# Lymphatus/caesium-clt

Measured on NVIDIA H100. Metric: megapixels/sec JPEG q=80 4K re-encode, higher is better.
Workload: dtype i32

## Files before the change

### caesium-clt_b200/csrc/jpeg_gpuenc.cu

```cuda
#include <cuda_runtime.h>
#include <cub/device/device_scan.cuh>
#include <cuda_pipeline.h>
#include <algorithm>
#include <chrono>
#include <cstring>
#include "jpeg_gpuenc.h"
#include "stream_wait.h"
#include "launch_timer.h"

namespace b200 {

using namespace ge;

__global__ void k_ge_groups(const Scan *__restrict__ scans, const uint32_t *__restrict__ meta, const int *__restrict__ evkey,
                            const int *__restrict__ prev, const uint32_t *__restrict__ tsum, uint32_t *__restrict__ gcount, uint32_t *__restrict__ hist)
{
    __shared__ uint32_t eob[16];
    const Scan s = scans[blockIdx.y];
    if (s.mode != MODE_AC_FIRST && s.mode != MODE_AC_REFINE) return;
    if ((int)(blockIdx.x * blockDim.x) > s.nblocks) return;
    if (threadIdx.x < 16) eob[threadIdx.x] = 0;
    __syncthreads();
    const int b = blockIdx.x * blockDim.x + threadIdx.x;
    if (b <= s.nblocks && (b == s.nblocks || meta_event(meta[s.unit_base + b]))) {
        int pg;
        if (b < s.nblocks) pg = prev[s.unit_base + b];
        else { const long long last = s.unit_base + s.nblocks - 1; pg = max(prev[last], evkey[last]); }
        const int pl = pg >= s.unit_base ? (int)(pg - s.unit_base) : -1;
        assign_groups(meta + s.unit_base, tsum + s.unit_base, s.nblocks, pl, b, gcount + s.unit_base,
                      [&](uint32_t c) { atomicAdd(&eob[eob_symbol(c) >> 4], 1u); });
    }
    __syncthreads();
    if (threadIdx.x < 16 && eob[threadIdx.x]) atomicAdd(&hist[((size_t)s.tab_base + 2 + s.tbl[0]) * 256 + (threadIdx.x << 4)], eob[threadIdx.x]);
}

__global__ void k_ge_tables(const uint32_t *__restrict__ hist, Table *__restrict__ tabs, DhtOut *__restrict__ dht, unsigned long long *__restrict__ tbits)
{
    __shared__ long long freq[257];
    __shared__ int codesize[257], others[257];
    __shared__ uint8_t bits[33];
    const int t = blockIdx.x, lane = threadIdx.x;
    const uint32_t *f = hist + (size_t)t * 256;
    for (int i = lane; i < 257; i += 32) { freq[i] = i < 256 ? (long long)f[i] : 1; codesize[i] = 0; others[i] = -1; }
    if (lane == 0) for (int i = 0; i < 33; i++) bits[i] = 0;
    __syncwarp();
    auto warp_argmin = [&](int exclude) {
        unsigned long long v = 1000000000ULL; int c = -1;
        for (int i = lane; i < 257; i += 32) { const unsigned long long fi = (unsigned long long)freq[i]; if (fi && fi <= v && i != exclude) { v = fi; c = i; } }
        const unsigned hi = (unsigned)(v >> 32), lo = (unsigned)v;
        const unsigned mhi = __reduce_min_sync(0xFFFFFFFFu, hi);
        const unsigned mlo = __reduce_min_sync(0xFFFFFFFFu, hi == mhi ? lo : 0xFFFFFFFFu);
        return __reduce_max_sync(0xFFFFFFFFu, (hi == mhi && lo == mlo) ? c : -1);
    };
    for (;;) {
        const int c1 = warp_argmin(-1);
        const int c2 = c1 < 0 ? -1 : warp_argmin(c1);
        if (c2 < 0) break;
        if (lane == 0) {
            int a = c1, b = c2;
            freq[a] += freq[b]; freq[b] = 0;
            codesize[a]++; while (others[a] >= 0) { a = others[a]; codesize[a]++; }
            others[a] = b;
            codesize[b]++; while (others[b] >= 0) { b = others[b]; codesize[b]++; }
        }
        __syncwarp();
    }
    if (lane == 0) {
        Table &T = tabs[t];
        for (int i = 0; i <= 256; i++) if (codesize[i]) bits[codesize[i] > 32 ? 32 : codesize[i]]++;
        for (int i = 32; i > 16; i--) while (bits[i] > 0) {
            int j = i - 2; while (bits[j] == 0) j--;
            bits[i] -= 2; bits[i - 1]++; bits[j + 1] += 2; bits[j]--;
        }
        int i = 16; while (i > 0 && bits[i] == 0) i--;
        if (i > 0) bits[i]--;
        int start[34];
        for (int l = 0; l < 34; l++) start[l] = 0;
        for (int s = 0; s <= 255; s++) if (codesize[s]) start[min(codesize[s], 32) + 1]++;
        for (int l = 1; l < 34; l++) start[l] += start[l - 1];
        const int p = start[33];
        for (int s = 0; s <= 255; s++) if (codesize[s]) T.vals[start[min(codesize[s], 32)]++] = (uint8_t)s;
        T.nvals = p;
        for (int k = 0; k < 17; k++) T.bits[k] = bits[k];
        for (int s = 0; s < 256; s++) T.code_len[s] = 0;
        uint32_t code = 0; int k = 0;
        for (int l = 1; l <= 16; l++) { for (int n = 0; n < bits[l]; n++, k++) T.code_len[T.vals[k]] = (code++ << 8) | (uint32_t)l; code <<= 1; }
        DhtOut &D = dht[t];
        D.nvals = p;
        for (int k2 = 0; k2 < 17; k2++) D.bits[k2] = bits[k2];
        for (int k2 = 0; k2 < p; k2++) D.vals[k2] = T.vals[k2];
    }
    __syncwarp();
    const int kind = (t & 3) >> 1;
    unsigned long long nb = 0;
    for (int i = lane; i < 256; i += 32) if (f[i]) nb += (unsigned long long)f[i] * ((tabs[t].code_len[i] & 0xFFu) + (unsigned)sym_extra_bits(kind, i));
    for (int d = 16; d; d >>= 1) nb += __shfl_xor_sync(0xFFFFFFFFu, nb, d);
    if (lane == 0) tbits[t] = nb;
}

__global__ void k_ge_scanout(const Scan *__restrict__ scans, int nscans, const unsigned long long *__restrict__ tbits, const uint32_t *__restrict__ corr,
                             uint32_t *__restrict__ total, ScanOut *__restrict__ so, uint32_t words_cap, uint32_t groups_cap, uint32_t *__restrict__ flags)
{
    const int lane = threadIdx.x;
    uint32_t wbase = 0, gbase = 0, abase = 0;
    for (int c0 = 0; c0 < nscans; c0 += 32) {
        const int i = c0 + lane;
        uint32_t tb = 0, na = 0;
        if (i < nscans) {
            tb = (uint32_t)(tbits[4 * i] + tbits[4 * i + 1] + tbits[4 * i + 2] + tbits[4 * i + 3] + corr[i]);
            na = scans[i].nruns ? (tb + 31) / 32 + scans[i].nruns : 0;
        }
        const uint32_t nbytes = (tb + 7) / 8, ng = (nbytes + 15) / 16, nw = i < nscans ? (tb + 31) / 32 + 1 : 0;
        uint32_t wi = nw, gi = i < nscans ? ng : 0, ai = na;
        for (int d = 1; d < 32; d <<= 1) {
            const uint32_t a = __shfl_up_sync(0xFFFFFFFFu, wi, d), b = __shfl_up_sync(0xFFFFFFFFu, gi, d), c = __shfl_up_sync(0xFFFFFFFFu, ai, d);
            if (lane >= d) { wi += a; gi += b; ai += c; }
        }
        if (i < nscans) {
            total[i] = tb;
            ScanOut o; o.total_bits = tb; o.nbytes = nbytes; o.ngroups = ng; o.group_base = gbase + gi - ng; o.word_base = wbase + wi - nw; o.arena_base = abase + ai - na;
            so[i] = o;
        }
        wbase += __shfl_sync(0xFFFFFFFFu, wi, 31); gbase += __shfl_sync(0xFFFFFFFFu, gi, 31); abase += __shfl_sync(0xFFFFFFFFu, ai, 31);
    }
    __syncwarp();
    const bool ovf = wbase > words_cap || gbase > groups_cap;
    if (lane == 0) { flags[0] = ovf ? 1u : 0u; flags[1] = wbase; flags[2] = gbase; flags[3] = 0; flags[4] = 0; }
    if (ovf) for (int i = lane; i < nscans; i += 32) { so[i].total_bits = 0; so[i].nbytes = 0; so[i].ngroups = 0; so[i].group_base = 0; so[i].word_base = 0; so[i].arena_base = 0; }
}

__global__ void k_ge_zero(const Scan *__restrict__ scans, const ScanOut *__restrict__ so, uint32_t *__restrict__ words, uint32_t *__restrict__ arena)
{
    const ScanOut o = so[blockIdx.y];
    if (!o.total_bits) return;
    const uint32_t n = (o.total_bits + 31) / 32 + 1, nruns = (uint32_t)scans[blockIdx.y].nruns, na = nruns ? n - 1 + nruns : 0;
    uint32_t *w = words + o.word_base, *a = arena + o.arena_base;
    for (uint32_t i = blockIdx.x * blockDim.x + threadIdx.x; i < max(n, na); i += gridDim.x * blockDim.x) {
        if (i < n) w[i] = 0;
        if (i < na) a[i] = 0;
    }
}

constexpr int TILE_PITCH = 72;
typedef int16_t Tile[ENC_THREADS][TILE_PITCH];

__device__ __forceinline__ void stage_tile(Tile &tile, const BlockComp &bc, int i0, int nblk)
{
    const uint4 *src = reinterpret_cast<const uint4 *>(bc.coef + bc.comp_off + (long long)i0 * 64);
    const int n = min(ENC_THREADS, nblk - i0) * 8;
#pragma unroll
    for (int k = 0; k < 8; k++) { const int q = threadIdx.x + k * ENC_THREADS; if (q < n) __pipeline_memcpy_async(&tile[q >> 3][(q & 7) * 8], src + q, 16); }
    __pipeline_commit();
}
__device__ __forceinline__ void wait_tile()
{
    __pipeline_wait_prior(0);
    __syncthreads();
}

__device__ __forceinline__ void stage_visits(EncVisit *vis, const BlockComp &bc)
{
    if ((int)threadIdx.x < bc.nscan) vis[threadIdx.x] = bc.visit[threadIdx.x];
}
__device__ __forceinline__ BlockRef ref_of(const EncVisit &v, const BlockComp &bc, const Tile &tile, int i0, int row, int col)
{
    BlockRef r;
    r.blk = tile[threadIdx.x]; r.prev = nullptr; r.slot = 0;
    if (v.mode == MODE_SEQ || v.mode == MODE_DC_FIRST) {
        const int p = enc_dc_prev(bc, v.ns, row, col);
        if (p >= i0 && p < i0 + ENC_THREADS) r.prev = tile[p - i0];
        else if (p >= 0) r.prev = bc.coef + bc.comp_off + (long long)p * 64;
    }
    return r;
}

template <class T>
__device__ __forceinline__ KindTabs<T> kind_tabs(T *tab, const EncVisit &v) { return KindTabs<T>{tab + ENC_DC_ENTRY, tab + v.ac_entry}; }

__device__ __forceinline__ Masks3 load_masks(const Masks3 *__restrict__ masks, const BlockComp &bc, int i)
{
    const unsigned long long *q = reinterpret_cast<const unsigned long long *>(masks + bc.mask_base + i);
    Masks3 M;
    M.m[0] = __ldg(q); M.m[1] = __ldg(q + 1); M.m[2] = __ldg(q + 2);
    return M;
}

struct SmemHist {
    KindTabs<uint32_t> h;
    __device__ void sym(int kind, int, int symbol, int, unsigned) { atomicAdd((kind ? h.ac : h.dc) + symbol, 1u); }
    __device__ void raw64(int, unsigned long long) {}
};
__global__ void __launch_bounds__(ENC_THREADS) k_geb_classify(const BlockComp *__restrict__ comps, uint32_t *__restrict__ meta, int *__restrict__ evkey,
                                                              uint32_t *__restrict__ tail, Masks3 *__restrict__ masks, uint32_t *__restrict__ hist, uint32_t *__restrict__ corr)
{
    __shared__ __align__(16) Tile tile;
    __shared__ uint32_t h[ENC_TAB_ENTRIES];
    __shared__ EncVisit vis[ENC_MAX_VISITS];
    __shared__ uint32_t vcorr[ENC_MAX_VISITS];
    const BlockComp &bc = comps[blockIdx.y];
    const int nblk = bc.bw * bc.bh, i0 = blockIdx.x * ENC_THREADS, i = i0 + threadIdx.x;
    if (i0 >= nblk) return;
    stage_tile(tile, bc, i0, nblk);
    for (int k = threadIdx.x; k < ENC_TAB_ENTRIES; k += ENC_THREADS) h[k] = 0;
    if (threadIdx.x < ENC_MAX_VISITS) vcorr[threadIdx.x] = 0;
    stage_visits(vis, bc);
    wait_tile();
    if (i < nblk) {
        const int row = i / bc.bw, col = i - row * bc.bw;
        const Masks3 M = make_masks3(tile[threadIdx.x]);
        masks[bc.mask_base + i] = M;
        for (int j = 0; j < bc.nscan; j++) {
// ... 86 lines not shown
                                                          const uint32_t *__restrict__ flags, uint32_t *__restrict__ arena, uint32_t *__restrict__ cursor,
                                                          uint32_t *__restrict__ runlen, uint32_t *__restrict__ runpos)
{
    __shared__ __align__(16) Tile tile;
    __shared__ uint32_t tc[ENC_TAB_ENTRIES];
    __shared__ EncVisit vis[ENC_MAX_VISITS];
    __shared__ uint32_t vword[ENC_MAX_VISITS], vbit0[ENC_MAX_VISITS];
    __shared__ uint32_t slot[ENC_SLOT_WORDS][ENC_THREADS];
    __shared__ uint32_t wsum[ENC_THREADS / 32], run_word;
    if (flags[0]) return;
    const BlockComp &bc = comps[blockIdx.y];
    const int nblk = bc.bw * bc.bh, i0 = blockIdx.x * ENC_THREADS, i = i0 + threadIdx.x;
    if (i0 >= nblk) return;
    const bool live = i < nblk;
    stage_tile(tile, bc, i0, nblk);
    const Masks3 M = load_masks(masks, bc, min(i, nblk - 1));
    stage_visits(vis, bc);
    if ((int)threadIdx.x < bc.nscan) {
        const EncVisit &v = bc.visit[threadIdx.x];
        const ScanOut &o = so[v.scan];
        vword[threadIdx.x] = v.ns > 1 ? o.word_base : o.arena_base; vbit0[threadIdx.x] = v.ns > 1 ? bitoff[v.lu_base] : 0;
    }
    for (int k = threadIdx.x; k < ENC_TAB_ENTRIES; k += ENC_THREADS) {
        int symbol; const int t = enc_entry_table(bc, k, symbol);
        if (t >= 0) tc[k] = tabs[t].code_len[symbol];
    }
    wait_tile();
    const int row = i / bc.bw, col = i - row * bc.bw;
    auto orw = [&](long long w, uint32_t v) { if (v) atomicOr(&words[w], v); };
    auto stw = [&](long long w, uint32_t v) { words[w] = v; };
    auto ora = [&](long long w, uint32_t v) { if (v) atomicOr(&arena[w], v); };
    auto sta = [&](long long w, uint32_t v) { arena[w] = v; };
    auto sls = [&](long long w, uint32_t v) { if (w < ENC_SLOT_WORDS) slot[w][threadIdx.x] = v; };
    typedef KindTabs<const uint32_t> KT;
    for (int j = 0; j < bc.nscan; j++) {
        const EncVisit &v = vis[j];
        const int u = live ? enc_unit_of(bc, v.ns, row, col) : -1;
        if (v.ns > 1) {
            if (u < 0) continue;
            EmitSink<decltype(orw), decltype(stw), KT> sk(kind_tabs<const uint32_t>(tc, v), orw, stw, (long long)vword[j], (unsigned long long)(bitoff[v.lu_base + u] - vbit0[j]));
            gen_block_m(v, v.tbl, ref_of(v, bc, tile, i0, row, col), M, gcount[v.unit_base + u], sk);
            sk.finish();
            continue;
        }
        uint32_t nb = 0;
        if (u >= 0) {
            EmitSink<decltype(sls), decltype(sls), KT> sk(kind_tabs<const uint32_t>(tc, v), sls, sls, 0, 0);
            gen_block_m(v, v.tbl, ref_of(v, bc, tile, i0, row, col), M, gcount[v.unit_base + u], sk);
            sk.finish();
            nb = (uint32_t)sk.bits_written(0);
        }
        uint32_t L;
        const uint32_t off = cta_exclusive_sum(nb, wsum, L);
        if (threadIdx.x == 0) {
            const uint32_t a = vword[j] + atomicAdd(&cursor[v.scan], (L + 31) / 32);
            run_word = a; runlen[v.run_base + blockIdx.x] = L; runpos[v.run_base + blockIdx.x] = a;
        }
        __syncthreads();
        const unsigned long long at = (unsigned long long)run_word * 32 + off;
        if (nb <= ENC_SLOT_WORDS * 32) place_bits([&](long long k) { return slot[k][threadIdx.x]; }, nb, at, ora, sta);
        else {
            EmitSink<decltype(ora), decltype(sta), KT> sk(kind_tabs<const uint32_t>(tc, v), ora, sta, 0, at);
            gen_block_m(v, v.tbl, ref_of(v, bc, tile, i0, row, col), M, gcount[v.unit_base + u], sk);
            sk.finish();
        }
    }
}

constexpr int PLACE_THREADS = 128;
__global__ void __launch_bounds__(PLACE_THREADS) k_ge_place(const Scan *__restrict__ scans, const ScanOut *__restrict__ so, const uint32_t *__restrict__ runlen,
                                                            const uint32_t *__restrict__ runoff, const uint32_t *__restrict__ runpos, const uint32_t *__restrict__ arena,
                                                            uint32_t *__restrict__ words, const uint32_t *__restrict__ flags)
{
    if (flags[0]) return;
    const int nruns = scans[blockIdx.y].nruns, x = blockIdx.x * (PLACE_THREADS / 32) + (threadIdx.x >> 5);
    if (x >= nruns) return;
    const int r0 = scans[blockIdx.y].run_base, r = r0 + x;
    const uint32_t *src = arena + runpos[r];
    uint32_t *dst = words + so[blockIdx.y].word_base;
    place_bits([&](long long k) { return src[k]; }, runlen[r], runoff[r] - runoff[r0],
               [&](long long w, uint32_t v) { atomicOr(&dst[w], v); }, [&](long long w, uint32_t v) { dst[w] = v; }, threadIdx.x & 31, 32);
}

__device__ __forceinline__ uint32_t scan_byte(const uint32_t *__restrict__ w, uint32_t i, uint32_t nbytes, uint32_t total_bits)
{
    uint32_t b = (w[i >> 2] >> (24 - 8 * (i & 3))) & 0xFF;
    if (i == nbytes - 1 && (total_bits & 7)) b |= (1u << (8 - (total_bits & 7))) - 1u;
    return b;
}

__global__ void k_ge_ffcount(const ScanOut *__restrict__ so, int nscans, const uint32_t *__restrict__ words, uint32_t *__restrict__ ffcount, uint32_t groups_cap,
                             const uint32_t *__restrict__ flags)
{
    if ((int)blockIdx.y == nscans) {
        const uint32_t used = flags[0] ? 0u : flags[2];
        for (uint32_t g = used + blockIdx.x * blockDim.x + threadIdx.x; g < groups_cap; g += gridDim.x * blockDim.x) ffcount[g] = 0;
        return;
    }
    const ScanOut o = so[blockIdx.y];
    const uint32_t *w = words + o.word_base;
    for (uint32_t g = blockIdx.x * blockDim.x + threadIdx.x; g < o.ngroups; g += gridDim.x * blockDim.x) {
        uint32_t n = 0;
        for (uint32_t i = g * 16; i < g * 16 + 16 && i < o.nbytes; i++) n += scan_byte(w, i, o.nbytes, o.total_bits) == 0xFF;
        ffcount[o.group_base + g] = n;
    }
}

__global__ void k_ge_layout(const ScanOut *__restrict__ so, int scans_per_image, int nimages, const uint32_t *__restrict__ ffcount, const uint32_t *__restrict__ ffoff,
                            uint32_t *__restrict__ out_off, uint32_t *__restrict__ out_len, uint32_t out_image_stride, uint32_t *__restrict__ flags)
{
    const int im = blockIdx.x * blockDim.x + threadIdx.x;
    if (im >= nimages) return;
    uint32_t off = 0;
    for (int k = 0; k < scans_per_image; k++) {
        const int si = im * scans_per_image + k;
        const ScanOut o = so[si];
        uint32_t ff = 0;
        if (o.ngroups) { const uint32_t lastg = o.group_base + o.ngroups - 1; ff = ffoff[lastg] + ffcount[lastg] - ffoff[o.group_base]; }
        out_off[si] = off; out_len[si] = o.nbytes + ff;
        off += o.nbytes + ff;
    }
    atomicMax(&flags[3], off);
    if (off > out_image_stride) atomicOr(&flags[4], 1u);
}

__global__ void k_ge_scatter(const ScanOut *__restrict__ so, const uint32_t *__restrict__ words, const uint32_t *__restrict__ ffoff,
                             const uint32_t *__restrict__ out_off, uint8_t *__restrict__ out, int scans_per_image, size_t out_image_stride, const uint32_t *__restrict__ flags)
{
    if (flags[4]) return;
    const ScanOut o = so[blockIdx.y];
    const uint32_t *w = words + o.word_base;
    uint8_t *base = out + (size_t)(blockIdx.y / scans_per_image) * out_image_stride + out_off[blockIdx.y];
    for (uint32_t g = blockIdx.x * blockDim.x + threadIdx.x; g < o.ngroups; g += gridDim.x * blockDim.x) {
        uint8_t *dst = base + (size_t)g * 16 + (ffoff[o.group_base + g] - ffoff[o.group_base]);
        for (uint32_t i = g * 16; i < g * 16 + 16 && i < o.nbytes; i++) {
            const uint32_t b = scan_byte(w, i, o.nbytes, o.total_bits);
            *dst++ = (uint8_t)b;
            if (b == 0xFF) *dst++ = 0;
        }
    }
}

__global__ void k_ge_fill_dummy(int16_t *__restrict__ coef, long long comp_off, int bw, int bh, int rbw, int rbh, int hs)
{
    const int i = blockIdx.x * blockDim.x + threadIdx.x;
    if (i >= bw * bh) return;
    const int row = i / bw, col = i - row * bw;
    if (row < rbh && col < rbw) return;
    int r = row, c = col;
    while (r >= rbh || c >= rbw) { if (r >= rbh) { c = (c / hs) * hs + hs - 1; r--; } else c = rbw - 1; }
    int16_t *base = coef + comp_off;
    int16_t *dst = base + ((long long)row * bw + col) * 64;
    const int16_t dc = base[((long long)r * bw + c) * 64];
    for (int k = 1; k < 64; k++) dst[k] = 0;
    dst[0] = dc;
}

static inline size_t align_up(size_t v, size_t a) { return (v + a - 1) / a * a; }
static inline int cdiv(long long a, long long b) { return (int)((a + b - 1) / b); }

GpuEncoder::~GpuEncoder()
{
    if (ev_sizes) cudaEventDestroy((cudaEvent_t)ev_sizes);
}

bool GpuEncoder::size_back_buffers(size_t image_bytes, std::string &err)
{
    const int NS = (int)plan.scans.size();
    auto grow = [&](auto &buf, size_t need) { return buf.reserve(need, Grow::Pow2Half, err, &generation); };
    auto grow_arena = [&]() { return grow(d_arena, ((size_t)words_cap + (size_t)plan.total_runs) * 4 + 64); };
    if (nimg != cap_nimg) { cap_nimg = nimg; est_image_bytes = 0; }
    if (image_bytes <= est_image_bytes && words_cap) return grow_arena();
    est_image_bytes = image_bytes + image_bytes / 8;
    image_bytes = est_image_bytes;
    words_cap = (uint32_t)std::min<size_t>((size_t)nimg * (image_bytes / 4 + 1) + 2 * (size_t)NS + 64, 0xFFFFFF00u);
    groups_cap = (uint32_t)((size_t)words_cap / 4 + NS + 1);
    out_stride = align_up(image_bytes + image_bytes / 8 + 1024, 256);
    if (!grow_arena() || !grow(d_words, (size_t)words_cap * 4 + 64) || !grow(d_ffcount, (size_t)groups_cap * 4 + 4) || !grow(d_ffoff, (size_t)groups_cap * 4 + 4) ||
        !grow(d_out, out_stride * nimg)) return false;
    size_t tb3 = 0; cub::DeviceScan::ExclusiveSum((void *)nullptr, tb3, d_ffcount.get(), d_ffoff.get(), (int)groups_cap, (cudaStream_t)0);
    return grow(d_temp, tb3 + 256);
}

bool GpuEncoder::prepare(const JpegGeom &g, bool progressive, int16_t *const *d_coefs, int nimages, void *stream_, size_t out_bytes_hint, std::string &err)
{
    cudaStream_t st = (cudaStream_t)stream_;
    geom = g; prog = progressive;
    std::vector<const int16_t *> bases(d_coefs, d_coefs + nimages);
    coef_bases.assign(d_coefs, d_coefs + nimages);
    gpuenc_plan(g, progressive, bases.data(), nimages, plan);
    nimg = nimages;
    const int NS = (int)plan.scans.size();
    const long long U = plan.total_units, LU = std::max(plan.total_lunits, 1ll);
    const int R = std::max(plan.total_runs, 1);
    if (U >= (1ll << 31)) { err = "batch too large for the entropy encoder"; return false; }
    overflow = false;
    for (auto &sc_ : plan.scans) if (!masks_cover(sc_.mode, sc_.Al)) { err = "scan script outside the device encoder's mask range"; overflow = true; return false; }
    if (!plan.on_chip) { err = "scan script outside the device encoder's on-chip table slots"; overflow = true; return false; }
    if (!ev_sizes) { cudaEvent_t e; CU(cudaEventCreateWithFlags(&e, cudaEventDisableTiming | (stream_wait_mode() == 0 ? 0 : cudaEventBlockingSync))); ev_sizes = e; }
    auto grow = [&](auto &buf, size_t need) { return buf.reserve(need, Grow::Pow2Half, err, &generation); };
    const int NC = (int)plan.comps.size();
    if (!grow(d_scans, NS * sizeof(Scan)) || !grow(d_comps, NC * sizeof(BlockComp)) ||
        !grow(d_meta, U * 4) || !grow(d_evkey, U * 4) || !grow(d_prev, U * 4) || !grow(d_tail, U * 4) || !grow(d_tsum, U * 4) ||
        !grow(d_gcount, U * 4) || !grow(d_bitlen, LU * 4) || !grow(d_bitoff, LU * 4) || !grow(d_corr, (size_t)NS * 4) || !grow(d_tbits, (size_t)NS * 4 * 8) ||
        !grow(d_cursor, (size_t)NS * 4) || !grow(d_runlen, (size_t)R * 4) || !grow(d_runoff, (size_t)R * 4) || !grow(d_runpos, (size_t)R * 4) ||
        !grow(d_hist, (size_t)NS * 4 * 256 * 4) || !grow(d_tabs, (size_t)NS * 4 * sizeof(Table)) || !grow(d_dht, (size_t)NS * 4 * sizeof(DhtOut)) ||
        !grow(d_total, (size_t)NS * 4) || !grow(d_so, (size_t)NS * sizeof(ScanOut)) || !grow(d_outoff, (size_t)NS * 4) || !grow(d_outlen, (size_t)NS * 4) ||
        !grow(d_flags, 64) || !grow(d_masks, (size_t)plan.total_comp_blocks * sizeof(Masks3))) return false;
    o_scans = 0; o_total = o_scans + align_up((size_t)NS * sizeof(Scan), 256); o_outlen = o_total + align_up((size_t)NS * 4, 256);
    o_dht = o_outlen + align_up((size_t)NS * 4, 256); o_comps = o_dht + align_up((size_t)NS * 4 * sizeof(DhtOut), 256);
    o_flags = o_comps + align_up((size_t)NC * sizeof(BlockComp), 256);
    const size_t small_bytes = o_flags + 256;
    if (!grow(h_small, small_bytes)) return false;
    size_t tb1 = 0, tb2 = 0, tb3 = 0, tb4 = 0;
    cub::DeviceScan::ExclusiveScan((void *)nullptr, tb1, d_evkey.get(), d_prev.get(), cub::Max(), -1, (int)U, st);
    cub::DeviceScan::ExclusiveSum((void *)nullptr, tb2, d_tail.get(), d_tsum.get(), (int)U, st);
    cub::DeviceScan::ExclusiveSum((void *)nullptr, tb3, d_bitlen.get(), d_bitoff.get(), (int)LU, st);
    cub::DeviceScan::ExclusiveSum((void *)nullptr, tb4, d_runlen.get(), d_runoff.get(), R, st);
    if (!grow(d_temp, std::max(std::max(tb1, tb2), std::max(tb3, tb4)) + 256)) return false;
    const size_t coef_bytes = (size_t)g.total_coefs * 2;
    if (coef_bytes != learned_for) { learned_for = coef_bytes; learned_image_bytes = 0; }
    size_t est = out_bytes_hint ? out_bytes_hint / nimages + out_bytes_hint / nimages / 4 : coef_bytes / 3;
    est = std::max(est, learned_image_bytes + learned_image_bytes / 8) + 8192;
    est = std::min(est, coef_bytes * 2 + (size_t)plan.scans_per_image * 64 + 8192);
    if (!size_back_buffers(est, err)) return false;
    memcpy(h_small + o_scans, plan.scans.data(), NS * sizeof(Scan));
    memcpy(h_small + o_comps, plan.comps.data(), NC * sizeof(BlockComp));
    (void)st;
    return true;
}

bool GpuEncoder::upload(void *stream_, std::string &err)
{
    cudaStream_t st = (cudaStream_t)stream_;
    const int NS = (int)plan.scans.size(), NC = (int)plan.comps.size();
    CU(cudaMemcpyAsync(d_scans, h_small + o_scans, NS * sizeof(Scan), cudaMemcpyHostToDevice, st));
    CU(cudaMemcpyAsync(d_comps, h_small + o_comps, NC * sizeof(BlockComp), cudaMemcpyHostToDevice, st));
    return true;
}

unsigned long long GpuEncoder::signature() const
{
    unsigned long long h = 1469598103934665603ull;
    auto mix = [&](unsigned long long v) { h = (h ^ v) * 1099511628211ull; };
    mix((unsigned long long)nimg); mix((unsigned long long)plan.scans.size()); mix((unsigned long long)plan.comps.size()); mix((unsigned long long)plan.total_units);
    mix((unsigned long long)plan.max_comp_blocks); mix((unsigned long long)plan.scans_per_image); mix(words_cap); mix(groups_cap); mix(out_stride); mix(generation);
    mix((unsigned long long)geom.width); mix((unsigned long long)geom.height); mix(prog ? 1 : 0);
    for (int c = 0; c < geom.ncomp; c++) { mix((unsigned long long)geom.bw[c]); mix((unsigned long long)geom.bh[c]); mix((unsigned long long)geom.rbw[c]); mix((unsigned long long)geom.rbh[c]); mix((unsigned long long)geom.hs[c]); }
    for (auto pb : coef_bases) mix((unsigned long long)(uintptr_t)pb);
    int max_units = 0; for (auto &sc : plan.scans) max_units = std::max(max_units, sc.nblocks);
    mix((unsigned long long)max_units);
    mix((unsigned long long)plan.total_lunits); mix((unsigned long long)plan.total_runs); mix((unsigned long long)plan.max_runs);
    return h;
}

bool GpuEncoder::enqueue_sizes(void *stream_, std::string &err)
{
    cudaStream_t st = (cudaStream_t)stream_;
    const int NS = (int)plan.scans.size();
    uint32_t *h_total = reinterpret_cast<uint32_t *>(h_small + o_total), *h_flags = reinterpret_cast<uint32_t *>(h_small + o_flags);
    k_ge_scanout<<<1, 32, 0, st>>>(d_scans, NS, d_tbits, d_corr, d_total, d_so, words_cap, groups_cap, d_flags);
    LT_MARK("k_ge_scanout");
    CU(cudaMemcpyAsync(h_total, d_total, (size_t)NS * 4, cudaMemcpyDeviceToHost, st));
    CU(cudaMemcpyAsync(h_flags, d_flags, 12, cudaMemcpyDeviceToHost, st));
    LT_MARK("copy");
    return true;
}
bool GpuEncoder::mark_sizes(void *stream_, std::string &err)
{
    CU(cudaEventRecord((cudaEvent_t)ev_sizes, (cudaStream_t)stream_));
    return true;
}

bool GpuEncoder::enqueue_back(void *stream_, std::string &err)
{
    cudaStream_t st = (cudaStream_t)stream_;
    const int NS = (int)plan.scans.size(), NC = (int)plan.comps.size();
    uint32_t *h_flags = reinterpret_cast<uint32_t *>(h_small + o_flags);
    const dim3 gb(cdiv(plan.max_comp_blocks, ENC_THREADS), NC);
    int n = 6;
    if (plan.total_lunits) {
        bool dc_only = true;
        for (auto &sc : plan.scans) if (sc.ns > 1 && sc.mode != MODE_DC_FIRST) dc_only = false;
        if (dc_only) {
            k_geb_len_dc<<<dim3(cdiv(plan.max_comp_blocks, LEN_DC_THREADS), NC), LEN_DC_THREADS, 0, st>>>(d_comps, d_tabs, d_bitlen);
            LT_MARK("k_geb_len_dc");
        } else {
            k_geb_len<<<gb, ENC_THREADS, 0, st>>>(d_comps, d_gcount, d_tabs, d_bitlen, d_masks);
            LT_MARK("k_geb_len");
        }
        size_t tb = d_temp.capacity();
        cub::DeviceScan::ExclusiveSum(d_temp, tb, d_bitlen.get(), d_bitoff.get(), (int)plan.total_lunits, st);
        LT_MARK("cub_scan");
        n += 2;
    }
    CU(cudaMemsetAsync(d_cursor, 0, (size_t)NS * 4, st));
    LT_MARK("memset");
    k_ge_zero<<<dim3(64, NS), 256, 0, st>>>(d_scans, d_so, d_words, d_arena);
    LT_MARK("k_ge_zero");
    k_geb_emit<<<gb, ENC_THREADS, 0, st>>>(d_comps, d_gcount, d_tabs, d_bitoff, d_words, d_masks, d_so, d_flags, d_arena, d_cursor, d_runlen, d_runpos);
    LT_MARK("k_geb_emit");
    if (plan.total_runs) {
        size_t tb = d_temp.capacity();
        cub::DeviceScan::ExclusiveSum(d_temp, tb, d_runlen.get(), d_runoff.get(), plan.total_runs, st);
        LT_MARK("cub_scan");
        k_ge_place<<<dim3(cdiv(plan.max_runs, PLACE_THREADS / 32), NS), PLACE_THREADS, 0, st>>>(d_scans, d_so, d_runlen, d_runoff, d_runpos, d_arena, d_words, d_flags);
        LT_MARK("k_ge_place");
        n += 2;
    }
    k_ge_ffcount<<<dim3(32, NS + 1), 128, 0, st>>>(d_so, NS, d_words, d_ffcount, groups_cap, d_flags);
    LT_MARK("k_ge_ffcount");
    size_t tb = d_temp.capacity();
    cub::DeviceScan::ExclusiveSum(d_temp, tb, d_ffcount.get(), d_ffoff.get(), (int)groups_cap, st);
    LT_MARK("cub_scan");
    k_ge_layout<<<cdiv(nimg, 64), 64, 0, st>>>(d_so, plan.scans_per_image, nimg, d_ffcount, d_ffoff, d_outoff, d_outlen, (uint32_t)out_stride, d_flags);
    LT_MARK("k_ge_layout");
    k_ge_scatter<<<dim3(32, NS), 128, 0, st>>>(d_so, d_words, d_ffoff, d_outoff, d_out, plan.scans_per_image, out_stride, d_flags);
    LT_MARK("k_ge_scatter");
    CU(cudaMemcpyAsync(h_small + o_outlen, d_outlen, (size_t)NS * 4, cudaMemcpyDeviceToHost, st));
    CU(cudaMemcpyAsync(h_small + o_dht, d_dht, (size_t)NS * 4 * sizeof(DhtOut), cudaMemcpyDeviceToHost, st));
    CU(cudaMemcpyAsync(h_flags + 4, d_flags, 32, cudaMemcpyDeviceToHost, st));
    CU(cudaGetLastError());
    launches += n;
    return true;
}

bool GpuEncoder::enqueue(void *stream_, bool fill_dummy, std::string &err)
{
    return enqueue_front(stream_, fill_dummy, err) && enqueue_sizes(stream_, err) && mark_sizes(stream_, err) && enqueue_back(stream_, err);
}

bool GpuEncoder::enqueue_front(void *stream_, bool fill_dummy, std::string &err)
{
    cudaStream_t st = (cudaStream_t)stream_;
    const JpegGeom &g = geom;
    const int NS = (int)plan.scans.size(), NC = (int)plan.comps.size();
    const long long U = plan.total_units;
    int max_units = 0; for (auto &s : plan.scans) max_units = std::max(max_units, s.nblocks);
    launches = 0;
    const dim3 gb(cdiv(plan.max_comp_blocks, ENC_THREADS), NC);
    if (fill_dummy) {
        for (int im = 0; im < nimg; im++) for (int cc = 0; cc < g.ncomp; cc++) {
            if (g.rbw[cc] == g.bw[cc] && g.rbh[cc] == g.bh[cc]) continue;
            k_ge_fill_dummy<<<cdiv((long long)g.bw[cc] * g.bh[cc], 256), 256, 0, st>>>(coef_bases[im], g.comp_offset[cc], g.bw[cc], g.bh[cc], g.rbw[cc], g.rbh[cc], g.hs[cc]);
            LT_MARK("k_ge_fill_dummy");
            launches++;
        }
    }
    const dim3 gu1(cdiv(max_units + 1, 128), NS);
    CU(cudaMemsetAsync(d_hist, 0, (size_t)NS * 4 * 256 * 4, st));
    LT_MARK("memset");
    CU(cudaMemsetAsync(d_corr, 0, (size_t)NS * 4, st));
    LT_MARK("memset");
    k_geb_classify<<<gb, ENC_THREADS, 0, st>>>(d_comps, d_meta, d_evkey, d_tail, d_masks, d_hist, d_corr);
    LT_MARK("k_geb_classify");
    size_t tb = d_temp.capacity();
    cub::DeviceScan::ExclusiveScan(d_temp, tb, d_evkey.get(), d_prev.get(), cub::Max(), -1, (int)U, st);
    LT_MARK("cub_scan");
    tb = d_temp.capacity();
    cub::DeviceScan::ExclusiveSum(d_temp, tb, d_tail.get(), d_tsum.get(), (int)U, st);
    LT_MARK("cub_scan");
    CU(cudaMemsetAsync(d_gcount, 0, U * 4, st));
    LT_MARK("memset");
    k_ge_groups<<<gu1, 128, 0, st>>>(d_scans, d_meta, d_evkey, d_prev, d_tsum, d_gcount, d_hist);
    LT_MARK("k_ge_groups");
    k_ge_tables<<<NS * 4, 32, 0, st>>>(d_hist, d_tabs, d_dht, d_tbits);
    LT_MARK("k_ge_tables");
    launches += 5;
    CU(cudaGetLastError());
    return true;
}

bool GpuEncoder::finish(void *stream_, bool fetch, std::string &err)
{
    cudaStream_t st = (cudaStream_t)stream_;
    const int NS = (int)plan.scans.size(), spi = plan.scans_per_image;
    uint32_t *h_total = reinterpret_cast<uint32_t *>(h_small + o_total), *h_flags = reinterpret_cast<uint32_t *>(h_small + o_flags);
    uint32_t *h_outlen = reinterpret_cast<uint32_t *>(h_small + o_outlen);
    const DhtOut *h_dht = reinterpret_cast<const DhtOut *>(h_small + o_dht);
    for (int attempt = 0;; attempt++) {
        const auto tw0 = std::chrono::steady_clock::now();
        if (fetch) { CU(event_wait((cudaEvent_t)ev_sizes)); } else { CU(stream_wait(st)); }
        wait_sizes_ms = std::chrono::duration<double, std::milli>(std::chrono::steady_clock::now() - tw0).count();
        size_t img_max = 0, img = 0;
        for (int si = 0; si < NS; si++) { img += (h_total[si] + 7) / 8; if ((si + 1) % spi == 0) { img_max = std::max(img_max, img); img = 0; } }
        if (h_flags[0]) {
            if (attempt >= 3) { err = "entropy encoder could not size its buffers"; return false; }
            CU(stream_wait(st));
            if (!size_back_buffers(img_max + img_max / 16 + 4096, err)) return false;
            retries++;
            if (!enqueue_sizes(st, err) || !mark_sizes(st, err) || !enqueue_back(st, err)) return false;
            continue;
        }
        if (fetch) {
            copy_bytes = std::min(out_stride, align_up(img_max + img_max / 8 + 256, 256));
            if (!h_out.reserve(copy_bytes * nimg, Grow::Pow2Half, err, &generation)) return false;
            for (int im = 0; im < nimg; im++) CU(cudaMemcpyAsync(h_out + (size_t)im * copy_bytes, d_out + (size_t)im * out_stride, copy_bytes, cudaMemcpyDeviceToHost, st));
            CU(cudaGetLastError());
            const auto tw1 = std::chrono::steady_clock::now();
            CU(stream_wait(st));
// ... 46 lines not shown
```

### caesium-clt_b200/csrc/jpeg_gpuenc.h

```cpp
#pragma once
#include <cstdint>
#include <cstddef>
#include <string>
#include <vector>
#include "dev_buffer.h"
#include "jpeg_gpuenc_plan.h"

namespace b200 {

struct DhtOut { uint8_t bits[17]; uint8_t vals[256]; int32_t nvals; };
struct ScanOut { uint32_t total_bits, nbytes, ngroups, group_base, word_base, arena_base; };

class GpuEncoder {
public:
    GpuEncoder() = default;
    ~GpuEncoder();
    GpuEncoder(const GpuEncoder &) = delete;
    GpuEncoder &operator=(const GpuEncoder &) = delete;
    bool encode(const JpegGeom &g, bool progressive, int16_t *const *d_coefs, int nimages, void *stream, bool fill_dummy, std::string &err, size_t out_bytes_hint = 0);
    bool prepare(const JpegGeom &g, bool progressive, int16_t *const *d_coefs, int nimages, void *stream, size_t out_bytes_hint, std::string &err);
    bool upload(void *stream, std::string &err);
    bool enqueue(void *stream, bool fill_dummy, std::string &err);
    bool enqueue_front(void *stream, bool fill_dummy, std::string &err);
    bool enqueue_sizes(void *stream, std::string &err);
    bool mark_sizes(void *stream, std::string &err);
    bool enqueue_back(void *stream, std::string &err);
    unsigned long long signature() const;
    bool finish(void *stream, bool fetch, std::string &err);
    int retries = 0;
    double wait_sizes_ms = 0, wait_final_ms = 0;
    std::vector<EncodedScan> results;
    GpuEncPlan plan;
    bool overflow = false;
    int launches = 0;
private:
    bool size_back_buffers(size_t image_bytes, std::string &err);
    unsigned long long generation = 0;
    int cap_nimg = 0;
    int nimg = 0;
    JpegGeom geom; bool prog = false;
    std::vector<int16_t *> coef_bases;
    void *ev_sizes = nullptr;
    uint32_t words_cap = 0, groups_cap = 0;
    size_t est_image_bytes = 0, learned_image_bytes = 0, learned_for = 0;
    DeviceBuffer<uint32_t> d_flags;
    size_t o_scans = 0, o_total = 0, o_outlen = 0, o_dht = 0, o_comps = 0, o_flags = 0;
    DeviceBuffer<ge::Scan> d_scans;
    DeviceBuffer<BlockComp> d_comps;
    DeviceBuffer<uint32_t> d_meta, d_tail, d_tsum, d_gcount;
    DeviceBuffer<uint32_t> d_bitlen, d_bitoff;
    DeviceBuffer<uint32_t> d_corr;
    DeviceBuffer<unsigned long long> d_tbits;
    DeviceBuffer<uint32_t> d_cursor, d_runlen, d_runoff, d_runpos, d_arena;
    DeviceBuffer<int> d_evkey, d_prev;
    DeviceBuffer<uint32_t> d_hist;
    DeviceBuffer<ge::Table> d_tabs;
    DeviceBuffer<DhtOut> d_dht;
    DeviceBuffer<uint32_t> d_total;
    DeviceBuffer<ScanOut> d_so;
    DeviceBuffer<uint32_t> d_words;
    DeviceBuffer<ge::Masks3> d_masks;
    DeviceBuffer<uint32_t> d_ffcount, d_ffoff;
    DeviceBuffer<uint32_t> d_outoff, d_outlen;
    DeviceBuffer<uint8_t> d_out;
    DeviceBuffer<uint8_t> d_temp;
    PinnedBuffer<uint8_t> h_small;
    PinnedBuffer<uint8_t> h_out;
    size_t out_stride = 0, copy_bytes = 0;
};

}
```

Baseline: 45790.

## Replace per-group FF stuffing scan with chunked counts and shared-memory staged scatter

Byte stuffing now counts 0xFF bytes per 16-byte group using a vector uint4 load and a SWAR popcount. Each kernel block reduces its count to one per-chunk total, which removes the global per-group ffcount/ffoff arrays and the cub ExclusiveSum launch. The scatter kernel builds the stuffed bytes in shared memory with a CTA prefix sum and writes them out as aligned 32-bit stores instead of byte-by-byte global writes. Word bases are padded to multiples of 4 so the uint4 loads stay aligned, at the cost of a slightly larger words buffer and extra syncthreads in the scatter loop.

```diff
diff --git a/caesium-clt_b200/csrc/jpeg_gpuenc.cu b/caesium-clt_b200/csrc/jpeg_gpuenc.cu
--- a/caesium-clt_b200/csrc/jpeg_gpuenc.cu
+++ b/caesium-clt_b200/csrc/jpeg_gpuenc.cu
@@ -5,6 +5,7 @@
 #include <chrono>
 #include <cstring>
 #include "jpeg_gpuenc.h"
+#include "jpeg_gpuenc_stuff_core.h"
 #include "stream_wait.h"
 #include "launch_timer.h"
 
@@ -99,10 +100,10 @@
 }
 
 __global__ void k_ge_scanout(const Scan *__restrict__ scans, int nscans, const unsigned long long *__restrict__ tbits, const uint32_t *__restrict__ corr,
-                             uint32_t *__restrict__ total, ScanOut *__restrict__ so, uint32_t words_cap, uint32_t groups_cap, uint32_t *__restrict__ flags)
+                             uint32_t *__restrict__ total, ScanOut *__restrict__ so, uint32_t words_cap, uint32_t *__restrict__ flags)
 {
     const int lane = threadIdx.x;
-    uint32_t wbase = 0, gbase = 0, abase = 0;
+    uint32_t wbase = 0, abase = 0;
     for (int c0 = 0; c0 < nscans; c0 += 32) {
         const int i = c0 + lane;
         uint32_t tb = 0, na = 0;
@@ -110,23 +111,23 @@
             tb = (uint32_t)(tbits[4 * i] + tbits[4 * i + 1] + tbits[4 * i + 2] + tbits[4 * i + 3] + corr[i]);
             na = scans[i].nruns ? (tb + 31) / 32 + scans[i].nruns : 0;
         }
-        const uint32_t nbytes = (tb + 7) / 8, ng = (nbytes + 15) / 16, nw = i < nscans ? (tb + 31) / 32 + 1 : 0;
-        uint32_t wi = nw, gi = i < nscans ? ng : 0, ai = na;
+        const uint32_t nbytes = (tb + 7) / 8, nw = i < nscans ? ((tb + 31) / 32 + 1 + 3) & ~3u : 0;
+        uint32_t wi = nw, ai = na;
         for (int d = 1; d < 32; d <<= 1) {
-            const uint32_t a = __shfl_up_sync(0xFFFFFFFFu, wi, d), b = __shfl_up_sync(0xFFFFFFFFu, gi, d), c = __shfl_up_sync(0xFFFFFFFFu, ai, d);
-            if (lane >= d) { wi += a; gi += b; ai += c; }
+            const uint32_t a = __shfl_up_sync(0xFFFFFFFFu, wi, d), c = __shfl_up_sync(0xFFFFFFFFu, ai, d);
+            if (lane >= d) { wi += a; ai += c; }
         }
         if (i < nscans) {
             total[i] = tb;
-            ScanOut o; o.total_bits = tb; o.nbytes = nbytes; o.ngroups = ng; o.group_base = gbase + gi - ng; o.word_base = wbase + wi - nw; o.arena_base = abase + ai - na;
+            ScanOut o; o.total_bits = tb; o.nbytes = nbytes; o.word_base = wbase + wi - nw; o.arena_base = abase + ai - na;
             so[i] = o;
         }
-        wbase += __shfl_sync(0xFFFFFFFFu, wi, 31); gbase += __shfl_sync(0xFFFFFFFFu, gi, 31); abase += __shfl_sync(0xFFFFFFFFu, ai, 31);
+        wbase += __shfl_sync(0xFFFFFFFFu, wi, 31); abase += __shfl_sync(0xFFFFFFFFu, ai, 31);
     }
     __syncwarp();
-    const bool ovf = wbase > words_cap || gbase > groups_cap;
-    if (lane == 0) { flags[0] = ovf ? 1u : 0u; flags[1] = wbase; flags[2] = gbase; flags[3] = 0; flags[4] = 0; }
-    if (ovf) for (int i = lane; i < nscans; i += 32) { so[i].total_bits = 0; so[i].nbytes = 0; so[i].ngroups = 0; so[i].group_base = 0; so[i].word_base = 0; so[i].arena_base = 0; }
+    const bool ovf = wbase > words_cap;
+    if (lane == 0) { flags[0] = ovf ? 1u : 0u; flags[1] = wbase; flags[3] = 0; flags[4] = 0; }
+    if (ovf) for (int i = lane; i < nscans; i += 32) { so[i].total_bits = 0; so[i].nbytes = 0; so[i].word_base = 0; so[i].arena_base = 0; }
 }
 
 __global__ void k_ge_zero(const Scan *__restrict__ scans, const ScanOut *__restrict__ so, uint32_t *__restrict__ words, uint32_t *__restrict__ arena)
@@ -379,62 +380,77 @@
                [&](long long w, uint32_t v) { atomicOr(&dst[w], v); }, [&](long long w, uint32_t v) { dst[w] = v; }, threadIdx.x & 31, 32);
 }
 
-__device__ __forceinline__ uint32_t scan_byte(const uint32_t *__restrict__ w, uint32_t i, uint32_t nbytes, uint32_t total_bits)
-{
-    uint32_t b = (w[i >> 2] >> (24 - 8 * (i & 3))) & 0xFF;
-    if (i == nbytes - 1 && (total_bits & 7)) b |= (1u << (8 - (total_bits & 7))) - 1u;
-    return b;
-}
-
-__global__ void k_ge_ffcount(const ScanOut *__restrict__ so, int nscans, const uint32_t *__restrict__ words, uint32_t *__restrict__ ffcount, uint32_t groups_cap,
-                             const uint32_t *__restrict__ flags)
-{
-    if ((int)blockIdx.y == nscans) {
-        const uint32_t used = flags[0] ? 0u : flags[2];
-        for (uint32_t g = used + blockIdx.x * blockDim.x + threadIdx.x; g < groups_cap; g += gridDim.x * blockDim.x) ffcount[g] = 0;
-        return;
-    }
+constexpr int STUFF_THREADS = ENC_THREADS;
+constexpr int STUFF_CHUNKS = 32;
+static_assert(STUFF_CHUNKS <= STUFF_THREADS, "k_ge_scatter sums the chunks before its own with one thread each");
+__device__ __forceinline__ ScanGroup load_scan_group(const uint32_t *w, uint32_t g) { const uint4 q = reinterpret_cast<const uint4 *>(w)[g]; return ScanGroup{{q.x, q.y, q.z, q.w}}; }
+
+__global__ void __launch_bounds__(STUFF_THREADS) k_ge_ffcount(const ScanOut *__restrict__ so, const uint32_t *__restrict__ words, uint32_t *__restrict__ chunkff)
+{
+    __shared__ uint32_t wsum[STUFF_THREADS / 32];
     const ScanOut o = so[blockIdx.y];
     const uint32_t *w = words + o.word_base;
-    for (uint32_t g = blockIdx.x * blockDim.x + threadIdx.x; g < o.ngroups; g += gridDim.x * blockDim.x) {
-        uint32_t n = 0;
-        for (uint32_t i = g * 16; i < g * 16 + 16 && i < o.nbytes; i++) n += scan_byte(w, i, o.nbytes, o.total_bits) == 0xFF;
-        ffcount[o.group_base + g] = n;
-    }
-}
-
-__global__ void k_ge_layout(const ScanOut *__restrict__ so, int scans_per_image, int nimages, const uint32_t *__restrict__ ffcount, const uint32_t *__restrict__ ffoff,
-                            uint32_t *__restrict__ out_off, uint32_t *__restrict__ out_len, uint32_t out_image_stride, uint32_t *__restrict__ flags)
-{
-    const int im = blockIdx.x * blockDim.x + threadIdx.x;
-    if (im >= nimages) return;
+    uint32_t g0, g1;
+    stuff_chunk(o.nbytes, blockIdx.x, STUFF_CHUNKS, STUFF_THREADS, g0, g1);
+    uint32_t n = 0;
+    for (uint32_t g = g0 + threadIdx.x; g < g1; g += STUFF_THREADS) {
+        ScanGroup q = load_scan_group(w, g);
+        stuff_group(q, g, o.nbytes, o.total_bits);
+        n += stuff_ff_count(q);
+    }
+    uint32_t total;
+    cta_exclusive_sum(n, wsum, total);
+    if (threadIdx.x == 0) chunkff[blockIdx.y * STUFF_CHUNKS + blockIdx.x] = total;
+}
+
+constexpr int LAYOUT_THREADS = 256;
+__global__ void __launch_bounds__(LAYOUT_THREADS) k_ge_layout(const ScanOut *__restrict__ so, int scans_per_image, const uint32_t *__restrict__ chunkff,
+                                                              uint32_t *__restrict__ out_off, uint32_t *__restrict__ out_len, uint32_t out_image_stride, uint32_t *__restrict__ flags)
+{
+    extern __shared__ uint32_t slen[];
+    const int lane = threadIdx.x & 31, s0 = blockIdx.x * scans_per_image;
+    for (int k = threadIdx.x >> 5; k < scans_per_image; k += LAYOUT_THREADS / 32) {
+        uint32_t ff = 0;
+        for (int x = lane; x < STUFF_CHUNKS; x += 32) ff += chunkff[(s0 + k) * STUFF_CHUNKS + x];
+        ff = __reduce_add_sync(0xFFFFFFFFu, ff);
+        if (lane == 0) slen[k] = so[s0 + k].nbytes + ff;
+    }
+    __syncthreads();
+    if (threadIdx.x) return;
     uint32_t off = 0;
-    for (int k = 0; k < scans_per_image; k++) {
-        const int si = im * scans_per_image + k;
-        const ScanOut o = so[si];
-        uint32_t ff = 0;
-        if (o.ngroups) { const uint32_t lastg = o.group_base + o.ngroups - 1; ff = ffoff[lastg] + ffcount[lastg] - ffoff[o.group_base]; }
-        out_off[si] = off; out_len[si] = o.nbytes + ff;
-        off += o.nbytes + ff;
-    }
+    for (int k = 0; k < scans_per_image; k++) { out_off[s0 + k] = off; out_len[s0 + k] = slen[k]; off += slen[k]; }
     atomicMax(&flags[3], off);
     if (off > out_image_stride) atomicOr(&flags[4], 1u);
 }
 
-__global__ void k_ge_scatter(const ScanOut *__restrict__ so, const uint32_t *__restrict__ words, const uint32_t *__restrict__ ffoff,
-                             const uint32_t *__restrict__ out_off, uint8_t *__restrict__ out, int scans_per_image, size_t out_image_stride, const uint32_t *__restrict__ flags)
-{
+__global__ void __launch_bounds__(STUFF_THREADS) k_ge_scatter(const ScanOut *__restrict__ so, const uint32_t *__restrict__ words, const uint32_t *__restrict__ chunkff,
+                                                              const uint32_t *__restrict__ out_off, uint8_t *__restrict__ out, int scans_per_image, size_t out_image_stride,
+                                                              const uint32_t *__restrict__ flags)
+{
+    __shared__ uint32_t sbuf[STUFF_THREADS * 8 + 1];
+    __shared__ uint32_t wsum[STUFF_THREADS / 32];
     if (flags[4]) return;
     const ScanOut o = so[blockIdx.y];
+    uint32_t g0, g1;
+    stuff_chunk(o.nbytes, blockIdx.x, STUFF_CHUNKS, STUFF_THREADS, g0, g1);
+    if (g0 >= g1) return;
     const uint32_t *w = words + o.word_base;
-    uint8_t *base = out + (size_t)(blockIdx.y / scans_per_image) * out_image_stride + out_off[blockIdx.y];
-    for (uint32_t g = blockIdx.x * blockDim.x + threadIdx.x; g < o.ngroups; g += gridDim.x * blockDim.x) {
-        uint8_t *dst = base + (size_t)g * 16 + (ffoff[o.group_base + g] - ffoff[o.group_base]);
-        for (uint32_t i = g * 16; i < g * 16 + 16 && i < o.nbytes; i++) {
-            const uint32_t b = scan_byte(w, i, o.nbytes, o.total_bits);
-            *dst++ = (uint8_t)b;
-            if (b == 0xFF) *dst++ = 0;
-        }
+    uint8_t *img = out + (size_t)(blockIdx.y / scans_per_image) * out_image_stride, *sb = reinterpret_cast<uint8_t *>(sbuf);
+    uint32_t ff_before;
+    cta_exclusive_sum(threadIdx.x < blockIdx.x ? chunkff[blockIdx.y * STUFF_CHUNKS + threadIdx.x] : 0u, wsum, ff_before);
+    uint32_t at = out_off[blockIdx.y] + g0 * 16 + ff_before;
+    for (uint32_t t0 = g0; t0 < g1; t0 += STUFF_THREADS) {
+        const uint32_t g = t0 + threadIdx.x;
+        ScanGroup q;
+        uint32_t n = 0, len = 0;
+        if (g < g1) { q = load_scan_group(w, g); n = stuff_group(q, g, o.nbytes, o.total_bits); len = n + stuff_ff_count(q); }
+        __syncthreads();
+        uint32_t L;
+        const uint32_t rel = cta_exclusive_sum(len, wsum, L), aligned = at & ~3u;
+        if (n) stuff_place_group(q, n, at - aligned + rel, sb);
+        __syncthreads();
+        stuff_store(sbuf, aligned, at, at + L, threadIdx.x, STUFF_THREADS, img);
+        at += L;
     }
 }
 
@@ -470,13 +486,9 @@
     if (image_bytes <= est_image_bytes && words_cap) return grow_arena();
     est_image_bytes = image_bytes + image_bytes / 8;
     image_bytes = est_image_bytes;
-    words_cap = (uint32_t)std::min<size_t>((size_t)nimg * (image_bytes / 4 + 1) + 2 * (size_t)NS + 64, 0xFFFFFF00u);
-    groups_cap = (uint32_t)((size_t)words_cap / 4 + NS + 1);
+    words_cap = (uint32_t)std::min<size_t>((size_t)nimg * (image_bytes / 4 + 1) + 5 * (size_t)NS + 64, 0xFFFFFF00u);
     out_stride = align_up(image_bytes + image_bytes / 8 + 1024, 256);
-    if (!grow_arena() || !grow(d_words, (size_t)words_cap * 4 + 64) || !grow(d_ffcount, (size_t)groups_cap * 4 + 4) || !grow(d_ffoff, (size_t)groups_cap * 4 + 4) ||
-        !grow(d_out, out_stride * nimg)) return false;
-    size_t tb3 = 0; cub::DeviceScan::ExclusiveSum((void *)nullptr, tb3, d_ffcount.get(), d_ffoff.get(), (int)groups_cap, (cudaStream_t)0);
-    return grow(d_temp, tb3 + 256);
+    return grow_arena() && grow(d_words, (size_t)words_cap * 4 + 64) && grow(d_out, out_stride * nimg);
 }
 
 bool GpuEncoder::prepare(const JpegGeom &g, bool progressive, int16_t *const *d_coefs, int nimages, void *stream_, size_t out_bytes_hint, std::string &err)
@@ -503,7 +515,7 @@
         !grow(d_cursor, (size_t)NS * 4) || !grow(d_runlen, (size_t)R * 4) || !grow(d_runoff, (size_t)R * 4) || !grow(d_runpos, (size_t)R * 4) ||
         !grow(d_hist, (size_t)NS * 4 * 256 * 4) || !grow(d_tabs, (size_t)NS * 4 * sizeof(Table)) || !grow(d_dht, (size_t)NS * 4 * sizeof(DhtOut)) ||
         !grow(d_total, (size_t)NS * 4) || !grow(d_so, (size_t)NS * sizeof(ScanOut)) || !grow(d_outoff, (size_t)NS * 4) || !grow(d_outlen, (size_t)NS * 4) ||
-        !grow(d_flags, 64) || !grow(d_masks, (size_t)plan.total_comp_blocks * sizeof(Masks3))) return false;
+        !grow(d_flags, 64) || !grow(d_masks, (size_t)plan.total_comp_blocks * sizeof(Masks3)) || !grow(d_chunkff, (size_t)NS * STUFF_CHUNKS * 4)) return false;
     o_scans = 0; o_total = o_scans + align_up((size_t)NS * sizeof(Scan), 256); o_outlen = o_total + align_up((size_t)NS * 4, 256);
     o_dht = o_outlen + align_up((size_t)NS * 4, 256); o_comps = o_dht + align_up((size_t)NS * 4 * sizeof(DhtOut), 256);
     o_flags = o_comps + align_up((size_t)NC * sizeof(BlockComp), 256);
@@ -541,7 +553,7 @@
     unsigned long long h = 1469598103934665603ull;
     auto mix = [&](unsigned long long v) { h = (h ^ v) * 1099511628211ull; };
     mix((unsigned long long)nimg); mix((unsigned long long)plan.scans.size()); mix((unsigned long long)plan.comps.size()); mix((unsigned long long)plan.total_units);
-    mix((unsigned long long)plan.max_comp_blocks); mix((unsigned long long)plan.scans_per_image); mix(words_cap); mix(groups_cap); mix(out_stride); mix(generation);
+    mix((unsigned long long)plan.max_comp_blocks); mix((unsigned long long)plan.scans_per_image); mix(words_cap); mix(out_stride); mix(generation);
     mix((unsigned long long)geom.width); mix((unsigned long long)geom.height); mix(prog ? 1 : 0);
     for (int c = 0; c < geom.ncomp; c++) { mix((unsigned long long)geom.bw[c]); mix((unsigned long long)geom.bh[c]); mix((unsigned long long)geom.rbw[c]); mix((unsigned long long)geom.rbh[c]); mix((unsigned long long)geom.hs[c]); }
     for (auto pb : coef_bases) mix((unsigned long long)(uintptr_t)pb);
@@ -556,10 +568,10 @@
     cudaStream_t st = (cudaStream_t)stream_;
     const int NS = (int)plan.scans.size();
     uint32_t *h_total = reinterpret_cast<uint32_t *>(h_small + o_total), *h_flags = reinterpret_cast<uint32_t *>(h_small + o_flags);
-    k_ge_scanout<<<1, 32, 0, st>>>(d_scans, NS, d_tbits, d_corr, d_total, d_so, words_cap, groups_cap, d_flags);
+    k_ge_scanout<<<1, 32, 0, st>>>(d_scans, NS, d_tbits, d_corr, d_total, d_so, words_cap, d_flags);
     LT_MARK("k_ge_scanout");
     CU(cudaMemcpyAsync(h_total, d_total, (size_t)NS * 4, cudaMemcpyDeviceToHost, st));
-    CU(cudaMemcpyAsync(h_flags, d_flags, 12, cudaMemcpyDeviceToHost, st));
+    CU(cudaMemcpyAsync(h_flags, d_flags, 8, cudaMemcpyDeviceToHost, st));
     LT_MARK("copy");
     return true;
 }
@@ -575,7 +587,7 @@
     const int NS = (int)plan.scans.size(), NC = (int)plan.comps.size();
     uint32_t *h_flags = reinterpret_cast<uint32_t *>(h_small + o_flags);
     const dim3 gb(cdiv(plan.max_comp_blocks, ENC_THREADS), NC);
-    int n = 6;
+    int n = 5;
     if (plan.total_lunits) {
         bool dc_only = true;
         for (auto &sc : plan.scans) if (sc.ns > 1 && sc.mode != MODE_DC_FIRST) dc_only = false;
@@ -605,14 +617,11 @@
         LT_MARK("k_ge_place");
         n += 2;
     }
-    k_ge_ffcount<<<dim3(32, NS + 1), 128, 0, st>>>(d_so, NS, d_words, d_ffcount, groups_cap, d_flags);
+    k_ge_ffcount<<<dim3(STUFF_CHUNKS, NS), STUFF_THREADS, 0, st>>>(d_so, d_words, d_chunkff);
     LT_MARK("k_ge_ffcount");
-    size_t tb = d_temp.capacity();
-    cub::DeviceScan::ExclusiveSum(d_temp, tb, d_ffcount.get(), d_ffoff.get(), (int)groups_cap, st);
-    LT_MARK("cub_scan");
-    k_ge_layout<<<cdiv(nimg, 64), 64, 0, st>>>(d_so, plan.scans_per_image, nimg, d_ffcount, d_ffoff, d_outoff, d_outlen, (uint32_t)out_stride, d_flags);
+    k_ge_layout<<<nimg, LAYOUT_THREADS, plan.scans_per_image * 4, st>>>(d_so, plan.scans_per_image, d_chunkff, d_outoff, d_outlen, (uint32_t)out_stride, d_flags);
     LT_MARK("k_ge_layout");
-    k_ge_scatter<<<dim3(32, NS), 128, 0, st>>>(d_so, d_words, d_ffoff, d_outoff, d_out, plan.scans_per_image, out_stride, d_flags);
+    k_ge_scatter<<<dim3(STUFF_CHUNKS, NS), STUFF_THREADS, 0, st>>>(d_so, d_words, d_chunkff, d_outoff, d_out, plan.scans_per_image, out_stride, d_flags);
     LT_MARK("k_ge_scatter");
     CU(cudaMemcpyAsync(h_small + o_outlen, d_outlen, (size_t)NS * 4, cudaMemcpyDeviceToHost, st));
     CU(cudaMemcpyAsync(h_small + o_dht, d_dht, (size_t)NS * 4 * sizeof(DhtOut), cudaMemcpyDeviceToHost, st));
diff --git a/caesium-clt_b200/csrc/jpeg_gpuenc.h b/caesium-clt_b200/csrc/jpeg_gpuenc.h
--- a/caesium-clt_b200/csrc/jpeg_gpuenc.h
+++ b/caesium-clt_b200/csrc/jpeg_gpuenc.h
@@ -9,7 +9,7 @@
 namespace b200 {
 
 struct DhtOut { uint8_t bits[17]; uint8_t vals[256]; int32_t nvals; };
-struct ScanOut { uint32_t total_bits, nbytes, ngroups, group_base, word_base, arena_base; };
+struct ScanOut { uint32_t total_bits, nbytes, word_base, arena_base; };
 
 class GpuEncoder {
 public:
@@ -41,7 +41,7 @@
     JpegGeom geom; bool prog = false;
     std::vector<int16_t *> coef_bases;
     void *ev_sizes = nullptr;
-    uint32_t words_cap = 0, groups_cap = 0;
+    uint32_t words_cap = 0;
     size_t est_image_bytes = 0, learned_image_bytes = 0, learned_for = 0;
     DeviceBuffer<uint32_t> d_flags;
     size_t o_scans = 0, o_total = 0, o_outlen = 0, o_dht = 0, o_comps = 0, o_flags = 0;
@@ -60,7 +60,7 @@
     DeviceBuffer<ScanOut> d_so;
     DeviceBuffer<uint32_t> d_words;
     DeviceBuffer<ge::Masks3> d_masks;
-    DeviceBuffer<uint32_t> d_ffcount, d_ffoff;
+    DeviceBuffer<uint32_t> d_chunkff;
     DeviceBuffer<uint32_t> d_outoff, d_outlen;
     DeviceBuffer<uint8_t> d_out;
     DeviceBuffer<uint8_t> d_temp;
diff --git a/caesium-clt_b200/csrc/jpeg_gpuenc_stuff_core.h b/caesium-clt_b200/csrc/jpeg_gpuenc_stuff_core.h
--- /dev/null
+++ b/caesium-clt_b200/csrc/jpeg_gpuenc_stuff_core.h
@@ -0,0 +1,63 @@
+#pragma once
+#include "jpeg_gpuenc_core.h"
+
+namespace b200 {
+namespace ge {
+
+struct ScanGroup { uint32_t w[4]; };
+
+GE_HD void stuff_chunk(uint32_t nbytes, uint32_t x, uint32_t nchunks, uint32_t tile, uint32_t &g0, uint32_t &g1)
+{
+    const uint32_t ng = (nbytes + 15) / 16, ntiles = (ng + tile - 1) / tile, per = (ntiles + nchunks - 1) / nchunks * tile;
+    g0 = x * per < ng ? x * per : ng;
+    g1 = (x + 1) * per < ng ? (x + 1) * per : ng;
+}
+
+GE_HD uint32_t stuff_group(ScanGroup &q, uint32_t g, uint32_t nbytes, uint32_t total_bits)
+{
+    const uint32_t left = nbytes - g * 16, n = left < 16 ? left : 16;
+    const uint32_t pad = (total_bits & 7) ? (1u << (8 - (total_bits & 7))) - 1u : 0u;
+#if defined(__CUDA_ARCH__)
+#pragma unroll
+#endif
+    for (int k = 0; k < 4; k++) {
+        const int nk = (int)n - 4 * k;
+        uint32_t w = nk <= 0 ? 0u : nk >= 4 ? q.w[k] : q.w[k] & ~(0xFFFFFFFFu >> (8 * nk));
+        if (n == left && nk >= 1 && nk <= 4) w |= pad << (8 * (4 - nk));
+        q.w[k] = w;
+    }
+    return n;
+}
+
+GE_HD uint32_t ff_bytes(uint32_t w)
+{
+    const uint32_t v = ~w;
+    return (uint32_t)popc64(~(((v & 0x7F7F7F7Fu) + 0x7F7F7F7Fu) | v) & 0x80808080u);
+}
+GE_HD uint32_t stuff_ff_count(const ScanGroup &q) { return ff_bytes(q.w[0]) + ff_bytes(q.w[1]) + ff_bytes(q.w[2]) + ff_bytes(q.w[3]); }
+
+GE_HD uint32_t stuff_place_group(const ScanGroup &q, uint32_t n, uint32_t o, uint8_t *sb)
+{
+#if defined(__CUDA_ARCH__)
+#pragma unroll
+#endif
+    for (int t = 0; t < 16; t++) {
+        if ((uint32_t)t >= n) break;
+        const uint32_t b = (q.w[t >> 2] >> (24 - 8 * (t & 3))) & 0xFFu;
+        sb[o++] = (uint8_t)b;
+        if (b == 0xFF) sb[o++] = 0;
+    }
+    return o;
+}
+
+GE_HD void stuff_store(const uint32_t *sbuf, uint32_t aligned, uint32_t first, uint32_t end, uint32_t tid, uint32_t nthreads, uint8_t *out)
+{
+    for (uint32_t a = aligned + 4 * tid; a < end; a += 4 * nthreads) {
+        const uint32_t w = sbuf[(a - aligned) >> 2];
+        if (a >= first && a + 4 <= end) *reinterpret_cast<uint32_t *>(out + a) = w;
+        else for (uint32_t t = 0; t < 4; t++) if (a + t >= first && a + t < end) out[a + t] = (uint8_t)(w >> (8 * t));
+    }
+}
+
+}
+}
```

Result: faster. 47250 (median of 6 runs) (+3.2%).
